# IvanPopov/video-flow-ml

Hardware: AMD Instinct MI355X
Metric: flow-fields/sec @1080p seq5 MOF_sintel (higher is better)
Workload: dtype mixed (per-layer MFMA count, f32 accumulate): {"corr": 1, "update_block.encoder.convf1": 1, "update_block.encoder.convf2": 1, "update_block.gru.convq1.iter": "2a", "update_block.gru.convzr1.iter": 1, "update_block.gru.convzr2.iter": 1, "update_block.mask.0": 1, "update_block.mask.2": 1, "update_bloc

## Files before the change

include/vfml.h:

```cpp
#ifndef VFML_H
#define VFML_H
#include <stddef.h>
#include <stdint.h>

#ifdef __cplusplus
extern "C" {
#endif

#define VFML_ABI_VERSION 26

enum {
  VFML_EPI_NONE = 0,
  VFML_EPI_RELU = 1,
  VFML_EPI_TANH = 2,
  VFML_EPI_SIGMOID = 3,
  VFML_EPI_TANH_RELU = 4,
  VFML_EPI_GRU_ZR = 5,
  VFML_EPI_GRU_Q = 6,
  VFML_EPI_ADD_AUX = 7,
};

enum { VFML_FMT_F32 = 0, VFML_FMT_S16 = 1,
       VFML_FMT_F16 = 2 };

// ... 48 lines not shown

int vfml_add_to_s16(const float* x, int64_t ldx, const float* aux, int64_t ld_aux, float* out, int64_t ld_out, int64_t rows,
                    int c, float scale, void* stream);

int vfml_transpose_split_f16(const float* src, int rows, int c, int ld, float scale, void* hi, void* lo, int kp,
                             void* stream);

int vfml_frames_to_nhwc4(const void* src, int kind, int n, int H, int W,
                         float scale, float shift, float* dst, void* stream);

int64_t vfml_instnorm_workspace_bytes(int n, int hw, int c);
int vfml_instnorm_stats(const float* x, int n, int hw, int c, float eps,
                        float* stats, void* workspace, void* stream);
int vfml_instnorm_apply(const float* x, const float* stats, const float* res,
                        const float* res_stats, int n, int hw, int c, float* out, int out_fmt, void* stream);

int vfml_avgpool2x2(const float* x, int n, int h, int w, int c, float* out, void* stream);

int vfml_corr_lookup(const float* const* pyr, const int32_t* hl, const int32_t* wl,
                     const int32_t* ld, int levels, int radius, int nmaps, int q_per_map,
                     const float* coords, int ld_coords, float* out, int ld_out, int out_fmt, int vol_fmt, int vol_tile,
                     void* stream);
#define VFML_VOL_F16_LEVELS(m) (0x100 | (m))

int vfml_corr_lookup_indirect(const float* const* table, const int32_t* hl, const int32_t* wl, const int32_t* ld,
                              int levels, int radius, int nmaps, int q_per_map, const float* coords, int ld_coords,
                              float* out, int ld_out, int out_fmt, int vol_fmt, int vol_tile, void* stream);
int vfml_corr_lookup_indirect_bidir(const float* const* table, const int32_t* hl, const int32_t* wl, const int32_t* ld,
                                    int levels, int radius, int nmaps, int q_per_map, const float* coords, int ld_coords,
                                    int dir_coords, float* out, int ld_out, int dir_out, int dir_tab, int out_fmt, int vol_fmt,
                                    int vol_tile, void* stream);
int vfml_ptr_table_set(void* table, const void* const* ptrs, int n, void* stream);

#define VFML_SEED_NONE 0
#define VFML_SEED_LOAD 1
#define VFML_SEED_STORE 2
int vfml_window_seed(const void* cells, int ncentres, int rows, int cols, float* state, int ld_state, int h_off, int mf_off,
                     int ld_ctx, void* stream);

int vfml_flow_rows7(const float* flow, int n, int h, int w, float* rows, void* stream);

int vfml_conv3x3_c64(const float* in, int ld_in, int n, int h, int w, const void* w_hi, const void* w_lo, int kp, float w_scale,
                     const float* bias, float* out, int ldo, double* stats_part, void* stream);

int vfml_flow_half(const float* flow, int n, int h, int w, const void* w1_hi, int kp1, float w1_scale, const float* b1,
                   const void* w2_hi, int kp2, float w2_scale, const float* b2, float* out, int ld_out, void* stream);

int vfml_tapsum3x3(const float* t, int ld_t, const float* bias, int n, int h, int w, float* out, int parts, int64_t part_stride,
                   void* stream);
int vfml_tapsum3x3_update(const float* t, int ld_t, const float* bias, int n, int h, int w, int parts, int64_t part_stride,
                          float* coords1, float* flow_a, int ld_a, float* flow_b, int ld_b, int fmt_b, void* stream);

int vfml_coords_update(float* coords1, const float* delta, int n, int h, int w,
                       float* flow_a, int ld_a, float* flow_b, int ld_b, int fmt_b, void* stream);
int vfml_coords_init(float* coords1, int n, int h, int w, void* stream);

int vfml_convex_upsample(const float* coords1, int ch, const float* mask, int ld_mask,
                         int h, int w, float* out, void* stream);
// ... 112 lines not shown
```

video-flow-ml_amd/vfml/csrc/enc_conv.hip:

```cpp
#include "conv_split_common.h"

namespace {

constexpr int EC_C = 64;
constexpr int EC_TH = 4, EC_TW = 32;
constexpr int EC_PR = EC_TH + 2, EC_PW = EC_TW + 2;
constexpr int EC_PIX = 272;
constexpr int EC_PATCH = EC_PR * EC_PW * EC_PIX;
constexpr int EC_VLD = EC_C + 4;
constexpr int EC_LDS = EC_PATCH;
constexpr int EC_K = 9 * EC_C;
constexpr int EC_NS = EC_K / 32;
static_assert(EC_TH * EC_TW * EC_VLD * 4 <= EC_PATCH, "the result tile fits where the patch was");

struct EncConvArgs {
  const char* in;
  const _Float16* whi; const _Float16* wlo;
  const float* bias;
  float* out; int ldo;
  double* stats_part;
  int ld_in, n, H, W, tiles_x, tiles_y;
  float w_inv;
};

__global__ __launch_bounds__(256, 2) void enc_conv3x3_c64_kernel(const EncConvArgs a) {
  extern __shared__ __attribute__((aligned(16))) char smem[];
  float* sV = reinterpret_cast<float*>(smem);

  const int t = threadIdx.x, lane = t & 63;
  const int wave = __builtin_amdgcn_readfirstlane(t >> 6);
  const int r4 = lane & 15, u4 = lane >> 4;
  const int tiles_img = a.tiles_x * a.tiles_y;
  const int total = a.n * tiles_img;

  h16x8 bh[EC_NS], bl[EC_NS];
  static_for<EC_NS>([&](auto sc) {
    constexpr int s = decltype(sc)::value;
    bh[s] = *reinterpret_cast<const h16x8*>(a.whi + (16 * wave + r4) * EC_K + s * 32 + u4 * 8);
    bl[s] = *reinterpret_cast<const h16x8*>(a.wlo + (16 * wave + r4) * EC_K + s * 32 + u4 * 8);
  });
  f32x4 bias4 = {0.f, 0.f, 0.f, 0.f};
  if (a.bias) bias4 = *reinterpret_cast<const f32x4*>(a.bias + 16 * wave + 4 * u4);

  for (int tile = blockIdx.x; tile < total; tile += gridDim.x) {
    const int img = tile / tiles_img, tl = tile - img * tiles_img;
    const int ty = tl / a.tiles_x, tx = tl - ty * a.tiles_x;
    const int oy0 = ty * EC_TH, ox0 = tx * EC_TW;

    constexpr int NPC = EC_PR * EC_PW * 16;
    constexpr int NPT = (NPC + 255) / 256;
    const __amdgpu_buffer_rsrc_t rin = __builtin_amdgcn_make_buffer_rsrc(
        const_cast<char*>(a.in) + (int64_t)img * a.H * a.W * a.ld_in * 4, 0, a.H * a.W * a.ld_in * 4, 0x00020000);
    u32x4 pv[NPT];
    static_for<NPT>([&](auto qc) {
      constexpr int q = decltype(qc)::value;
      const int c = min(t + 256 * q, NPC - 1);
      const int p = c >> 4, piece = c & 15;
      const int py = p / EC_PW, px = p - py * EC_PW;
      const int iy = oy0 - 1 + py, ix = ox0 - 1 + px;
      const bool ok = (unsigned)iy < (unsigned)a.H && (unsigned)ix < (unsigned)a.W;
      pv[q] = bload16(rin, ok ? ((iy * a.W + ix) * a.ld_in) * 4 + piece * 16 : (int)0x80000000);
    });
    __syncthreads();
    static_for<NPT>([&](auto qc) {
      constexpr int q = decltype(qc)::value;
      const int c = t + 256 * q;
      if (c < NPC) *reinterpret_cast<u32x4*>(smem + (c >> 4) * EC_PIX + (c & 15) * 16) = pv[q];
    });
    __syncthreads();

    f32x4 acc[8];
#pragma unroll
    for (int m = 0; m < 8; ++m) acc[m] = f32x4{0.f, 0.f, 0.f, 0.f};
    const char* al = smem + r4 * EC_PIX + u4 * 32;
    static_for<2>([&](auto hc) {
      constexpr int mh = decltype(hc)::value;
      static_for<EC_NS>([&](auto sc) {
        constexpr int s = decltype(sc)::value;
        constexpr int cb = s / 9, ky = (s % 9) / 3, kx = s % 3;
#pragma unroll
        for (int mm = 0; mm < 4; ++mm) {
          const int m = 4 * mh + mm;
// ... 33 lines not shown
          const double v = (double)g;
          s1 += v;
          s2 += v * v;
        }
        const int64_t chunk = (((int64_t)img * a.H + oy) * a.W + ox0) >> 5;
        double* o = a.stats_part + (chunk * EC_C + ch) * 2;
        o[0] = s1;
        o[1] = s2;
      }
    }
  }
}

}

extern "C" int vfml_conv3x3_c64(const float* in, int ld_in, int n, int h, int w, const void* w_hi, const void* w_lo, int kp,
                                float w_scale, const float* bias, float* out, int ldo, double* stats_part, void* stream) {
  VFML_REQUIRE(in && w_hi && w_lo && out && n > 0 && h > 0 && w > 0, "vfml_conv3x3_c64: bad argument");
  VFML_REQUIRE(w % EC_TW == 0, "vfml_conv3x3_c64: the image width must be a multiple of %d (got %d)", EC_TW, w);
  VFML_REQUIRE(kp == EC_K && w_scale > 0.f, "vfml_conv3x3_c64: weight planes [64][%d] (VFML_KORDER_CBLOCK), got row pitch %d", EC_K, kp);
  VFML_REQUIRE((reinterpret_cast<uintptr_t>(in) & 31u) == 0 && ld_in >= EC_C && ld_in % 8 == 0 && vfml_aligned16(w_hi) &&
                   vfml_aligned16(w_lo) && vfml_aligned16(bias) && vfml_aligned16(out) && ldo >= EC_C && ldo % 4 == 0 &&
                   (reinterpret_cast<uintptr_t>(stats_part) & 7u) == 0,
               "vfml_conv3x3_c64: a 32-byte aligned split-row input (ld_in %% 8 == 0), 16-byte aligned weights / bias / output "
               "(ldo %% 4 == 0)");
  EncConvArgs a;
  a.in = reinterpret_cast<const char*>(in); a.ld_in = ld_in;
  a.whi = reinterpret_cast<const _Float16*>(w_hi); a.wlo = reinterpret_cast<const _Float16*>(w_lo);
  a.bias = bias; a.out = out; a.ldo = ldo; a.stats_part = stats_part;
  a.n = n; a.H = h; a.W = w; a.tiles_x = w / EC_TW; a.tiles_y = (h + EC_TH - 1) / EC_TH;
  a.w_inv = 1.0f / w_scale;
  const int64_t total = (int64_t)n * a.tiles_x * a.tiles_y;
  VFML_REQUIRE(total < (1ll << 31) && (int64_t)h * w * ld_in * 4 < (1ll << 31), "vfml_conv3x3_c64: an image of the input must stay below 2 GiB");
  const int grid = (int)(total < 512 ? total : 512);
  hipLaunchKernelGGL(enc_conv3x3_c64_kernel, dim3(grid), dim3(256), EC_LDS, reinterpret_cast<hipStream_t>(stream), a);
  return vfml_check_launch("vfml_conv3x3_c64");
}
```

video-flow-ml_amd/vfml/csrc/norm_pool.hip:

```cpp
#include <stdlib.h>
#include "vfml_common.h"

namespace {

__global__ void frames_u8_kernel(const uint8_t* __restrict__ src, int64_t npx, float scale, float shift,
                                 f32x4* __restrict__ dst) {
  for (int64_t p = (int64_t)blockIdx.x * blockDim.x + threadIdx.x; p < npx; p += (int64_t)gridDim.x * blockDim.x) {
    const uint8_t* s = src + p * 3;
    f32x4 v;
    v[0] = scale * ((float)s[0] / 255.0f) + shift;
    v[1] = scale * ((float)s[1] / 255.0f) + shift;
    v[2] = scale * ((float)s[2] / 255.0f) + shift;
    v[3] = 0.f;
    dst[p] = v;
  }
}

__global__ void frames_f32_kernel(const float* __restrict__ src, int n, int64_t hw, float scale, float shift,
                                  f32x4* __restrict__ dst) {
  const int64_t npx = (int64_t)n * hw;
  for (int64_t p = (int64_t)blockIdx.x * blockDim.x + threadIdx.x; p < npx; p += (int64_t)gridDim.x * blockDim.x) {
    const int64_t f = p / hw, q = p - f * hw;
    const float* s = src + f * 3 * hw + q;
    f32x4 v;
// ... 121 lines not shown
    double* o = out + (((int64_t)nn * FOLD_SLICES + sl) * c + cg * 8 + ch) * 2;
    o[0] = ss;
    o[1] = qq;
  }
}

template <int MODE, bool S16>
__global__ void instnorm_apply_kernel(const f32x4* __restrict__ x, const float* __restrict__ stats,
                                      const f32x4* __restrict__ res, const float* __restrict__ rstats, int hw, int c,
                                      int64_t total4, f32x4* __restrict__ out) {
  const int cg = c >> 2;
  const int64_t per_n = (int64_t)hw * cg;
  for (int64_t i = (int64_t)blockIdx.x * blockDim.x + threadIdx.x; i < total4; i += (int64_t)gridDim.x * blockDim.x) {
    const int n = (int)(i / per_n);
    const int g = (int)(i % cg);
    const float* st = stats + ((int64_t)n * c + g * 4) * 2;
    const f32x4 v = x[i];
    f32x4 o;
#pragma unroll
    for (int e = 0; e < 4; ++e) o[e] = fmaxf((v[e] - st[2 * e]) * st[2 * e + 1], 0.f);
    const int64_t qoff = (i - g) * 16 + (g >> 1) * 32 + (g & 1) * 8;
    if (MODE == 1) {
      f32x4 rv;
      if (S16) {
        const char* u = reinterpret_cast<const char*>(res) + qoff;
        const vfml_h16x2 h0 = *reinterpret_cast<const vfml_h16x2*>(u), h1 = *reinterpret_cast<const vfml_h16x2*>(u + 4);
        const vfml_h16x2 l0 = *reinterpret_cast<const vfml_h16x2*>(u + 16), l1 = *reinterpret_cast<const vfml_h16x2*>(u + 20);
        rv[0] = (float)h0[0] + (float)l0[0];
        rv[1] = (float)h0[1] + (float)l0[1];
        rv[2] = (float)h1[0] + (float)l1[0];
        rv[3] = (float)h1[1] + (float)l1[1];
      } else {
        rv = res[i];
      }
#pragma unroll
      for (int e = 0; e < 4; ++e) o[e] = fmaxf(rv[e] + o[e], 0.f);
    } else if (MODE == 2) {
      const f32x4 rv = res[i];
      const float* rs = rstats + ((int64_t)n * c + g * 4) * 2;
#pragma unroll
      for (int e = 0; e < 4; ++e) o[e] = fmaxf((rv[e] - rs[2 * e]) * rs[2 * e + 1] + o[e], 0.f);
    }
    if (S16) {
      vfml_h16x2 h0, h1, l0, l1;
      vfml_split2(o[0], o[1], h0, l0);
      vfml_split2(o[2], o[3], h1, l1);
      char* u = reinterpret_cast<char*>(out) + qoff;
      uint2 hv, lv;
      hv.x = __builtin_bit_cast(unsigned, h0); hv.y = __builtin_bit_cast(unsigned, h1);
      lv.x = __builtin_bit_cast(unsigned, l0); lv.y = __builtin_bit_cast(unsigned, l1);
      *reinterpret_cast<uint2*>(u) = hv;
      *reinterpret_cast<uint2*>(u + 16) = lv;
    } else {
      out[i] = o;
    }
  }
}

__global__ void avgpool2x2_kernel(const f32x4* __restrict__ x, int h, int w, int cg, int ho, int wo, int64_t total4,
                                  f32x4* __restrict__ out) {
  for (int64_t i = (int64_t)blockIdx.x * blockDim.x + threadIdx.x; i < total4; i += (int64_t)gridDim.x * blockDim.x) {
    const int g = (int)(i % cg);
    int64_t p = i / cg;
    const int ox = (int)(p % wo);
    p /= wo;
    const int oy = (int)(p % ho);
    const int n = (int)(p / ho);
// ... 103 lines not shown
  const bool s16 = out_fmt == VFML_FMT_S16;
#define VFML_APPLY(MODE, S16, R, RS)                                                                                      \
  hipLaunchKernelGGL((instnorm_apply_kernel<MODE, S16>), g, b, 0, s, (const f32x4*)x, stats, (const f32x4*)(R), RS, hw, c, \
                     total4, (f32x4*)out)
  if (!res) {
    if (s16) VFML_APPLY(0, true, nullptr, nullptr); else VFML_APPLY(0, false, nullptr, nullptr);
  } else if (!res_stats) {
    if (s16) VFML_APPLY(1, true, res, nullptr); else VFML_APPLY(1, false, res, nullptr);
  } else {
    if (s16) VFML_APPLY(2, true, res, res_stats); else VFML_APPLY(2, false, res, res_stats);
  }
#undef VFML_APPLY
  return vfml_check_launch("vfml_instnorm_apply");
}

extern "C" int vfml_avgpool2x2(const float* x, int n, int h, int w, int c, float* out, void* stream) {
  VFML_REQUIRE(x && out, "vfml_avgpool2x2: null pointer");
  VFML_REQUIRE(n > 0 && h >= 2 && w >= 2 && c > 0 && c % 4 == 0, "vfml_avgpool2x2: bad shape");
  VFML_REQUIRE(vfml_aligned16(x) && vfml_aligned16(out), "vfml_avgpool2x2: alignment");
  const int ho = h / 2, wo = w / 2, cg = c / 4;
  const int64_t total4 = (int64_t)n * ho * wo * cg;
  hipLaunchKernelGGL(avgpool2x2_kernel, dim3(grid_for(total4, 256)), dim3(256), 0, reinterpret_cast<hipStream_t>(stream),
                     (const f32x4*)x, h, w, cg, ho, wo, total4, (f32x4*)out);
  return vfml_check_launch("vfml_avgpool2x2");
}
```

video-flow-ml_amd/vfml/csrc/vfml_common.h:

```cpp
#pragma once
#include <hip/hip_runtime.h>
#include <stdint.h>
#include <stdio.h>
#include <mutex>
#include <set>
#include <utility>
#include "../../../include/vfml.h"

typedef float f32x4 __attribute__((ext_vector_type(4)));
typedef float f32x16 __attribute__((ext_vector_type(16)));

typedef _Float16 vfml_h16x2 __attribute__((ext_vector_type(2)));

__device__ __forceinline__ void vfml_split2(float a, float b, vfml_h16x2& h, vfml_h16x2& l) {
  vfml_h16x2 hh = {(_Float16)a, (_Float16)b};
#if defined(__HIP_DEVICE_COMPILE__)
  unsigned hp = __builtin_bit_cast(unsigned, hh);
  asm volatile("" : "+v"(hp));
  hh = __builtin_bit_cast(vfml_h16x2, hp);
#endif
  h = hh;
  const vfml_h16x2 ll = {(_Float16)(a - (float)hh[0]), (_Float16)(b - (float)hh[1])};
  l = ll;
}

__device__ __forceinline__ double vfml_lds_f64(const double* p) {
#if defined(__HIP_DEVICE_COMPILE__)
  const uint2 u = *reinterpret_cast<const uint2*>(p);
  unsigned lo, hi;
  asm("v_mov_b32 %0, %1" : "=v"(lo) : "v"(u.x));
  asm("v_mov_b32 %0, %1" : "=v"(hi) : "v"(u.y));
  return __hiloint2double((int)hi, (int)lo);
#else
  return *p;
#endif
}

void vfml_set_error(const char* fmt, ...);
// ... 38 lines not shown
```

video-flow-ml_amd/vfml/hip.py:

```python
import ctypes
import os
import subprocess
from ctypes import POINTER, c_char_p, c_double, c_float, c_int, c_int32, c_int64, c_void_p

import torch

_HERE = os.path.dirname(os.path.abspath(__file__))
LIB_PATH = os.environ.get("VFML_LIB") or os.path.join(_HERE, "libvfml_hip.so")
CSRC = os.path.join(_HERE, "csrc")
SOURCES = ["api.hip", "conv_gemm.hip", "conv_gemm_split.hip", "conv_gemm_tapx.hip", "conv_split_plan.hip", "stem.hip", "flow_half.hip", "enc_conv.hip", "norm_pool.hip", "flow_ops.hip", "effects.hip", "correct.hip", "render.hip", "turbulence.hip", "resize.hip", "jpeg.hip", "jpeg_decode.hip", "jpeg_decode_sync.hip", "deflate.hip"]

STATS_ROWS_F32, STATS_ROWS_S16 = 128, 32
EPI_NONE, EPI_RELU, EPI_TANH, EPI_SIGMOID, EPI_TANH_RELU, EPI_GRU_ZR, EPI_GRU_Q, EPI_ADD_AUX = range(8)
FMT_F32, FMT_S16, FMT_F16 = 0, 1, 2


def vol_f16_levels(mask):
    return 0x100 | mask


def _vol_mask(vol_fmt, levels):
    return (15 if vol_fmt == FMT_F16 else (vol_fmt & 15 if vol_fmt & 0x100 else 0)) & ((1 << levels) - 1)

KORDER_TAP, KORDER_CBLOCK, KORDER_CBLOCK64 = 0, 1, 2
# ... 83 lines not shown
    L.vfml_transpose_split_f16.argtypes = [c_void_p, c_int, c_int, c_int, c_float, c_void_p, c_void_p, c_int, c_void_p]
    L.vfml_split_f16.argtypes = [c_void_p, c_int64, c_int, c_int, c_float, c_void_p, c_void_p, c_int, c_void_p]
    L.vfml_frames_to_nhwc4.argtypes = [c_void_p, c_int, c_int, c_int, c_int, c_float, c_float, c_void_p, c_void_p]
    L.vfml_instnorm_workspace_bytes.restype = c_int64
    L.vfml_instnorm_workspace_bytes.argtypes = [c_int, c_int, c_int]
    L.vfml_instnorm_stats.argtypes = [c_void_p, c_int, c_int, c_int, c_float, c_void_p, c_void_p, c_void_p]
    L.vfml_softmax_rows_f16.argtypes = [c_void_p, c_int64, c_int, c_int64, c_void_p, c_int64, c_float, c_void_p]
    L.vfml_transpose_to_s16.argtypes = [c_void_p, c_int, c_int, c_int, c_float, c_void_p, c_int64, c_void_p]
    L.vfml_add_to_s16.argtypes = [c_void_p, c_int64, c_void_p, c_int64, c_void_p, c_int64, c_int64, c_int, c_float, c_void_p]
    L.vfml_instnorm_finalize.argtypes = [c_void_p, c_int, c_int, c_int, c_int, c_float, c_void_p, c_void_p, c_int64, c_void_p]
    L.vfml_instnorm_finalize_workspace_bytes.restype = c_int64
    L.vfml_instnorm_finalize_workspace_bytes.argtypes = [c_int, c_int]
    L.vfml_stem7x7s2_chunks.argtypes = [c_int, c_int]
    L.vfml_stem7x7s2.argtypes = [c_void_p, c_int, c_int, c_int, c_void_p, c_void_p, c_float, c_void_p, c_void_p, c_void_p, c_void_p]
    L.vfml_instnorm_apply.argtypes = [c_void_p, c_void_p, c_void_p, c_void_p, c_int, c_int, c_int, c_void_p, c_int, c_void_p]
    L.vfml_avgpool2x2.argtypes = [c_void_p, c_int, c_int, c_int, c_int, c_void_p, c_void_p]
    L.vfml_corr_lookup.argtypes = [POINTER(c_void_p), POINTER(c_int32), POINTER(c_int32), POINTER(c_int32),
                                   c_int, c_int, c_int, c_int, c_void_p, c_int, c_void_p, c_int, c_int, c_int, c_int, c_void_p]
    L.vfml_corr_lookup_indirect.argtypes = [c_void_p, POINTER(c_int32), POINTER(c_int32), POINTER(c_int32),
                                            c_int, c_int, c_int, c_int, c_void_p, c_int, c_void_p, c_int, c_int, c_int, c_int,
                                            c_void_p]
    L.vfml_corr_lookup_indirect_bidir.argtypes = [c_void_p, POINTER(c_int32), POINTER(c_int32), POINTER(c_int32),
                                                  c_int, c_int, c_int, c_int, c_void_p, c_int, c_int, c_void_p, c_int, c_int,
                                                  c_int, c_int, c_int, c_int, c_void_p]
    L.vfml_ptr_table_set.argtypes = [c_void_p, POINTER(c_void_p), c_int, c_void_p]
    L.vfml_window_seed.argtypes = [c_void_p, c_int, c_int, c_int, c_void_p, c_int, c_int, c_int, c_int, c_void_p]
    L.vfml_tapsum3x3_update.argtypes = [c_void_p, c_int, c_void_p, c_int, c_int, c_int, c_int, ctypes.c_int64, c_void_p, c_void_p,
                                        c_int, c_void_p, c_int, c_int, c_void_p]
    L.vfml_conv3x3_c64.argtypes = [c_void_p, c_int, c_int, c_int, c_int, c_void_p, c_void_p, c_int, c_float, c_void_p, c_void_p,
                                   c_int, c_void_p, c_void_p]
    L.vfml_flow_half.argtypes = [c_void_p, c_int, c_int, c_int, c_void_p, c_int, c_float, c_void_p, c_void_p, c_int, c_float,
                                 c_void_p, c_void_p, c_int, c_void_p]
    L.vfml_coords_init.argtypes = [c_void_p, c_int, c_int, c_int, c_void_p]
    L.vfml_flow_rows7.argtypes = [c_void_p, c_int, c_int, c_int, c_void_p, c_void_p]
    L.vfml_tapsum3x3.argtypes = [c_void_p, c_int, c_void_p, c_int, c_int, c_int, c_void_p, c_int, ctypes.c_int64, c_void_p]
    L.vfml_coords_update.argtypes = [c_void_p, c_void_p, c_int, c_int, c_int, c_void_p, c_int, c_void_p, c_int,
                                     c_int, c_void_p]
    L.vfml_flow_lod.argtypes = [c_void_p, c_int, c_int, c_void_p, c_void_p]
    L.vfml_flow_encode.argtypes = [c_void_p, c_int, c_int, c_int, c_float, c_float, c_float, c_float, c_float, c_void_p,
                                   c_void_p]
    L.vfml_taa_blend.argtypes = [c_void_p, c_int, c_void_p, c_void_p, c_int, c_void_p, c_int, c_int, c_int, c_int, c_double,
                                 c_double, c_void_p]
    L.vfml_flow_quality_map.argtypes = [c_void_p, c_void_p, c_void_p, c_int, c_int, c_int, c_int, c_float, c_void_p, c_void_p]
    L.vfml_flow_correct_workspace_bytes.argtypes = [c_int, c_int]
    L.vfml_flow_correct_workspace_bytes.restype = ctypes.c_size_t
# ... 42 lines not shown
                                      c_void_p, c_void_p, c_void_p]
    L.vfml_convex_upsample.argtypes = [c_void_p, c_int, c_void_p, c_int, c_int, c_int, c_void_p, c_void_p]
    for name in EXPORTS:
        getattr(L, name)
    if L.vfml_abi_version() != 26:
        raise RuntimeError("libvfml_hip.so ABI version mismatch")
    _lib = L
    return L


EXPORTS = [
    "vfml_conv2d", "vfml_conv2d_split", "vfml_conv2d_variant", "vfml_conv2d_split_variant", "vfml_split_f16", "vfml_to_s16", "vfml_softmax_rows_s16", "vfml_softmax_rows_f16", "vfml_transpose_to_s16", "vfml_add_to_s16",
    "vfml_transpose_split_f16", "vfml_frames_to_nhwc4", "vfml_instnorm_workspace_bytes", "vfml_instnorm_stats",
    "vfml_instnorm_apply", "vfml_instnorm_finalize", "vfml_instnorm_finalize_workspace_bytes", "vfml_avgpool2x2", "vfml_corr_lookup", "vfml_corr_lookup_indirect", "vfml_corr_lookup_indirect_bidir",
    "vfml_ptr_table_set", "vfml_window_seed", "vfml_coords_update", "vfml_coords_init", "vfml_tapsum3x3", "vfml_tapsum3x3_update", "vfml_flow_rows7", "vfml_flow_half", "vfml_conv3x3_c64",
    "vfml_convex_upsample", "vfml_stem7x7s2", "vfml_stem7x7s2_chunks", "vfml_flow_lod", "vfml_flow_encode", "vfml_taa_blend", "vfml_flow_quality_map", "vfml_flow_correct_workspace_bytes", "vfml_flow_correct",
    "vfml_flow_colorize", "vfml_compose_frame", "vfml_flow_decode", "vfml_flow_diff_overlay",
    "vfml_flow_turbulence_workspace_bytes", "vfml_flow_turbulence_map", "vfml_resize_u8",
    "vfml_jpeg_workspace_bytes", "vfml_jpeg_scan_capacity", "vfml_jpeg_encode_rgb",
    "vfml_jpeg_decode_workspace_bytes", "vfml_jpeg_decode_rgb",
    "vfml_jpeg_decode_sync_workspace_bytes", "vfml_jpeg_decode_rgb_sync",
    "vfml_jpeg_decode_sampled_workspace_bytes", "vfml_jpeg_decode_rgb_sampled",
    "vfml_jpeg_decode_sync_sampled_workspace_bytes", "vfml_jpeg_decode_rgb_sync_sampled",
    "vfml_deflate_capacity", "vfml_deflate_workspace_bytes", "vfml_deflate_huffman",
    "vfml_inflate_workspace_bytes", "vfml_inflate_chunks",
    "vfml_last_error", "vfml_abi_version",
]


def _check(rc, what):
# ... 214 lines not shown
        raise ValueError(f"pack_stem_weight: a [64, 3|4, 7, 7] weight expected, got {tuple(w.shape)}")
    k = torch.zeros(cout, 7, 8, 4, device=device)
    k[:, :, :7, :cin] = w.permute(0, 2, 3, 1)
    sw = SplitWeight(cout, 224, device)
    return sw.fill(k.reshape(-1).contiguous(), scale=SplitWeight.auto_scale(float(w.abs().max())))


def stem7x7s2(frames, n, h, w, weight, bias, out, stats_part=None):
    if not isinstance(weight, SplitWeight) or weight.rows != 64 or weight.kp != 224:
        raise ValueError("stem7x7s2: weight must come from pack_stem_weight")
    _check(lib().vfml_stem7x7s2(_ptr(_dev(frames)), n, h, w, c_void_p(weight.hi.data_ptr()), c_void_p(weight.lo.data_ptr()),
                                weight.scale, _ptr(_dev(bias)) if bias is not None else None, _ptr(_dev(out)),
                                c_void_p(stats_part.data_ptr()) if stats_part is not None else None, _stream()), "vfml_stem7x7s2")


def instnorm_apply(x, stats, n, hw, c, out, res=None, res_stats=None, out_fmt=FMT_F32):
    _check(lib().vfml_instnorm_apply(_ptr(_dev(x)), _ptr(_dev(stats)), _ptr(res), _ptr(res_stats), n, hw, c,
                                     _ptr(_dev(out)), out_fmt, _stream()), "vfml_instnorm_apply")


def avgpool2x2(x, n, h, w, c, out):
    _check(lib().vfml_avgpool2x2(_ptr(_dev(x)), n, h, w, c, _ptr(_dev(out)), _stream()), "vfml_avgpool2x2")


def softmax_rows_s16(x, rows, cols, ld_in, out, ld_out, x_off=0, out_off=0, scale=1.0):
    _check(lib().vfml_softmax_rows_s16(_ptr(_dev(x), x_off), rows, cols, ld_in, _ptr(_dev(out), out_off), ld_out,
                                       float(scale), _stream()), "vfml_softmax_rows_s16")


class PlainWeight:
    lo = None
# ... 120 lines not shown
def flow_rows7(flow, n, h, w, rows):
    _check(lib().vfml_flow_rows7(_ptr(_dev(flow)), n, h, w, _ptr(_dev(rows)), _stream()), "vfml_flow_rows7")


def tapsum3x3(t, ld_t, bias, n, h, w, out, parts=1, part_stride=0):
    _check(lib().vfml_tapsum3x3(_ptr(_dev(t)), ld_t, _ptr(bias) if bias is not None else None, n, h, w, _ptr(_dev(out)),
                                parts, part_stride, _stream()), "vfml_tapsum3x3")


def conv3x3_c64(src, ld_in, n, h, w, weight, bias, out, ldo, stats_part=None, src_off=0):
    _check(lib().vfml_conv3x3_c64(_ptr(_dev(src), src_off), ld_in, n, h, w, c_void_p(weight.hi.data_ptr()),
                                  c_void_p(weight.lo.data_ptr()), weight.kp, weight.scale,
                                  _ptr(_dev(bias)) if bias is not None else None, _ptr(_dev(out)), ldo,
                                  c_void_p(stats_part.data_ptr()) if stats_part is not None else None, _stream()),
           "vfml_conv3x3_c64")


def flow_half(flow, n, h, w, w1, b1, w2, b2, out, ld_out, out_off=0):
    _check(lib().vfml_flow_half(_ptr(_dev(flow)), n, h, w, c_void_p(w1.hi.data_ptr()), w1.kp, w1.scale, _ptr(_dev(b1)),
                                c_void_p(w2.hi.data_ptr()), w2.kp, w2.scale, _ptr(_dev(b2)), _ptr(_dev(out), out_off), ld_out,
                                _stream()), "vfml_flow_half")


def tapsum3x3_update(t, ld_t, bias, n, h, w, coords1, parts=1, part_stride=0, flow_a=None, ld_a=0, flow_a_off=0, flow_b=None,
                     ld_b=0, flow_b_off=0, fmt_b=FMT_F32):
    _check(lib().vfml_tapsum3x3_update(_ptr(_dev(t)), ld_t, _ptr(bias) if bias is not None else None, n, h, w, parts, part_stride,
                                       _ptr(_dev(coords1)), _ptr(flow_a, flow_a_off), ld_a, _ptr(flow_b, flow_b_off), ld_b,
                                       fmt_b, _stream()), "vfml_tapsum3x3_update")


# ... 551 lines not shown
```

video-flow-ml_amd/vfml/network.py:

```python
import os

import torch
import torch.nn as nn

from . import hip
from .weights import conv_spec, corr_channel_subset, pack_conv_weight


def cor_pad(cor, split):
    return (cor + 15) // 16 * 16 if split else (cor + 3) // 4 * 4


def take_frames(src, idx):
    idx = list(idx)
    if all(b == a + 1 for a, b in zip(idx, idx[1:])):
        return src[idx[0]:idx[0] + len(idx)]
    return torch.stack([src[i] for i in idx])


class _Holder(nn.Module):

    def child(self, name):
        if name not in self._modules:
            self.add_module(name, _Holder())
# ... 330 lines not shown
            return
        st = self._graphs.get(key)
        if st is None:
            body()
            while len(self._graphs) >= self.GRAPHS_KEPT:
                self._graphs.pop(next(iter(self._graphs)))
            self._graphs[key] = "seen"
            return
        if st == "seen":
            g = torch.cuda.CUDAGraph()
            with torch.cuda.graph(g, capture_error_mode="thread_local"):
                body()
            self._graphs[key] = st = g
        st.replay()

    def _encoder(self, prefix, x, n, H, W, P, dev, out, ldo, out_off, epilogue, split, out_fmt=hip.FMT_F32):
        h2, w2 = H // 2, W // 2
        big = n * h2 * w2 * 64
        raw = self._buf("enc_raw", big, dev)
        raw2 = self._buf("enc_raw2", big, dev)
        act = [self._buf("enc_act0", big, dev), self._buf("enc_act1", big, dev), self._buf("enc_act2", big, dev)]
        st = self._buf("enc_stats", 3 * n * 128 * 2, dev)
        nws = hip.instnorm_workspace_bytes(n, h2 * w2, 128)
        ws = self._buf("enc_statws", (nws + 7) // 8, dev, torch.float64)

        def stats_of(t, hw, c, slot):
            s = st[slot * n * 128 * 2:]
            hip.instnorm_stats(t, n, hw, c, s, ws)
            return s

        split_prec = self._split()
        AF = hip.FMT_S16 if split_prec else hip.FMT_F32
        part_len = n * ((h2 * w2 + 31) // 32) * 64 * 2
        parts = self._buf("enc_part", 3 * part_len, dev, torch.float64) if split_prec else None
        fold_ws = self._buf("enc_foldws", min(n, 8) * 64 * 128 * 2, dev, torch.float64) if split_prec else None

        def conv_stats(src, c, hh_, ww_, name, planes, dst, slot, k, stride=1, pad=0, src_fmt=hip.FMT_F32):
            wgt, b = P[name]
            nm = self._nm(name) if split_prec else 3
            ho_, wo_ = (hh_ + 2 * pad - k) // stride + 1, (ww_ + 2 * pad - k) // stride + 1
            hw = ho_ * wo_
            rows = hip.STATS_ROWS_S16 if src_fmt == hip.FMT_S16 else hip.STATS_ROWS_F32
            if not (split_prec and (n == 1 or hw % rows == 0)):
                hip.conv2d(src, c, c, n, hh_, ww_, wgt, b, planes, k, k, dst, planes, stride=stride, pad_h=pad, pad_w=pad,
                           mfma=nm, in_fmt=src_fmt)
                return stats_of(dst, hw, planes, slot)
            chunks = (hw + rows - 1) // rows
            part = parts[slot * part_len:]
            if (c == 64 and planes == 64 and k == 3 and stride == 1 and pad == 1 and nm == 3 and src_fmt == hip.FMT_S16
                    and ww_ % 32 == 0 and getattr(wgt, "order", None) == hip.KORDER_CBLOCK and wgt.kp == 576 and wgt.lo is not None):
                hip.conv3x3_c64(src, c, n, hh_, ww_, wgt, b, dst, planes, stats_part=part)
            else:
                hip.conv2d(src, c, c, n, hh_, ww_, wgt, b, planes, k, k, dst, planes, stride=stride, pad_h=pad, pad_w=pad,
                           stats_part=part, mfma=nm, in_fmt=src_fmt)
            s = st[slot * n * 128 * 2:]
            hip.instnorm_finalize(part, n, chunks, planes, hw, s, workspace=fold_ws)
            return s

        stem = P.get(f"{prefix}.conv1.stem")
        if stem is not None and split_prec and self._nm(f"{prefix}.conv1") == 3:
            chunks = hip.stem_chunks(H, W)
            part = parts[0:]
            hip.stem7x7s2(x, n, H, W, stem[0], stem[1], raw, stats_part=part)
            s0 = st[0:]
            hip.instnorm_finalize(part, n, chunks, 64, h2 * w2, s0, workspace=fold_ws)
        else:
            s0 = conv_stats(x, 4, H, W, f"{prefix}.conv1", 64, raw, 0, 7, stride=2, pad=3)
        cur = act[0]
        hip.instnorm_apply(raw, s0, n, h2 * w2, 64, cur, out_fmt=AF)
        ch, hh, ww, ci = 64, h2, w2, 0
        for li, (planes, stride) in enumerate([(64, 1), (96, 2), (128, 2)], start=1):
            for bi in range(2):
                stv = stride if bi == 0 else 1
                ho, wo = (hh, ww) if stv == 1 else ((hh - 1) // 2 + 1, (ww - 1) // 2 + 1)
                name = f"{prefix}.layer{li}.{bi}"
                y = act[(ci + 1) % 3]
                nxt = act[(ci + 2) % 3]
                s1 = conv_stats(cur, ch, hh, ww, f"{name}.conv1", planes, raw, 0, 3, stride=stv, pad=1, src_fmt=AF)
                hip.instnorm_apply(raw, s1, n, ho * wo, planes, y, out_fmt=AF)
                s2 = conv_stats(y, planes, ho, wo, f"{name}.conv2", planes, raw, 1, 3, pad=1, src_fmt=AF)
                if stv != 1:
                    s3 = conv_stats(cur, ch, hh, ww, f"{name}.downsample.0", planes, raw2, 2, 1, stride=stv, src_fmt=AF)
                    hip.instnorm_apply(raw, s2, n, ho * wo, planes, nxt, res=raw2, res_stats=s3, out_fmt=AF)
                else:
                    hip.instnorm_apply(raw, s2, n, ho * wo, planes, nxt, res=cur, out_fmt=AF)
                cur, ci = nxt, (ci + 2) % 3
# ... 519 lines not shown
```

Measured before the change: 44.76.

## Fuse instance-norm+ReLU into encoder layer1 conv input loads

Adds a templated NORM variant of the 64-channel 3x3 encoder conv. It applies instance-norm and ReLU to raw fp32 inputs while staging them into LDS, splitting them into f16 hi/lo halves and zeroing the padding. The encoder's layer1 path now feeds raw conv outputs plus their stats straight into the next conv, and a new apply variant normalises the residual on the fly. This removes three standalone instnorm_apply passes over the activation map, at the cost of reading fp32 (twice the bytes of split storage) in the conv and extra ALU work in its load phase.

Result: no change. 45.12, median of 6 (+0.8%).

```diff
diff --git a/include/vfml.h b/include/vfml.h
--- a/include/vfml.h
+++ b/include/vfml.h
@@ -86,6 +86,8 @@
                         float* stats, void* workspace, void* stream);
 int vfml_instnorm_apply(const float* x, const float* stats, const float* res,
                         const float* res_stats, int n, int hw, int c, float* out, int out_fmt, void* stream);
+int vfml_instnorm_apply_normres(const float* x, const float* stats, const float* res, const float* res_stats, int n, int hw,
+                                int c, float* out, void* stream);
 
 int vfml_avgpool2x2(const float* x, int n, int h, int w, int c, float* out, void* stream);
 
@@ -114,6 +116,9 @@
 
 int vfml_conv3x3_c64(const float* in, int ld_in, int n, int h, int w, const void* w_hi, const void* w_lo, int kp, float w_scale,
                      const float* bias, float* out, int ldo, double* stats_part, void* stream);
+int vfml_conv3x3_c64_norm(const float* in, const float* in_stats, int ld_in, int n, int h, int w, const void* w_hi,
+                          const void* w_lo, int kp, float w_scale, const float* bias, float* out, int ldo, double* stats_part,
+                          void* stream);
 
 int vfml_flow_half(const float* flow, int n, int h, int w, const void* w1_hi, int kp1, float w1_scale, const float* b1,
                    const void* w2_hi, int kp2, float w2_scale, const float* b2, float* out, int ld_out, void* stream);
diff --git a/video-flow-ml_amd/vfml/csrc/enc_conv.hip b/video-flow-ml_amd/vfml/csrc/enc_conv.hip
--- a/video-flow-ml_amd/vfml/csrc/enc_conv.hip
+++ b/video-flow-ml_amd/vfml/csrc/enc_conv.hip
@@ -15,6 +15,7 @@
 
 struct EncConvArgs {
   const char* in;
+  const float* nstats;
   const _Float16* whi; const _Float16* wlo;
   const float* bias;
   float* out; int ldo;
@@ -23,6 +24,7 @@
   float w_inv;
 };
 
+template <bool NORM>
 __global__ __launch_bounds__(256, 2) void enc_conv3x3_c64_kernel(const EncConvArgs a) {
   extern __shared__ __attribute__((aligned(16))) char smem[];
   float* sV = reinterpret_cast<float*>(smem);
@@ -52,20 +54,37 @@
     const __amdgpu_buffer_rsrc_t rin = __builtin_amdgcn_make_buffer_rsrc(
         const_cast<char*>(a.in) + (int64_t)img * a.H * a.W * a.ld_in * 4, 0, a.H * a.W * a.ld_in * 4, 0x00020000);
     u32x4 pv[NPT];
+    unsigned inside = 0;
+    int ts = t;
+    if (NORM) asm volatile("" : "+v"(ts));
     static_for<NPT>([&](auto qc) {
       constexpr int q = decltype(qc)::value;
-      const int c = min(t + 256 * q, NPC - 1);
+      const int c = min(ts + 256 * q, NPC - 1);
       const int p = c >> 4, piece = c & 15;
       const int py = p / EC_PW, px = p - py * EC_PW;
       const int iy = oy0 - 1 + py, ix = ox0 - 1 + px;
       const bool ok = (unsigned)iy < (unsigned)a.H && (unsigned)ix < (unsigned)a.W;
       pv[q] = bload16(rin, ok ? ((iy * a.W + ix) * a.ld_in) * 4 + piece * 16 : (int)0x80000000);
+      if (NORM) inside |= (unsigned)ok << q;
     });
+    f32x4 mean = {0.f, 0.f, 0.f, 0.f}, rstd = mean;
+    if (NORM) vfml_load_stats4(a.nstats + ((int64_t)img * EC_C + 4 * (t & 15)) * 2, mean, rstd);
     __syncthreads();
     static_for<NPT>([&](auto qc) {
       constexpr int q = decltype(qc)::value;
       const int c = t + 256 * q;
-      if (c < NPC) *reinterpret_cast<u32x4*>(smem + (c >> 4) * EC_PIX + (c & 15) * 16) = pv[q];
+      if (c < NPC) {
+        if (NORM) {
+          vfml_s16quad s = vfml_norm_relu_split4(__builtin_bit_cast(f32x4, pv[q]), mean, rstd);
+          const unsigned keep = 0u - (inside >> q & 1u);
+          s.hi.x &= keep; s.hi.y &= keep; s.lo.x &= keep; s.lo.y &= keep;
+          char* u = smem + (c >> 4) * EC_PIX + ((c & 15) >> 1) * 32 + (c & 1) * 8;
+          *reinterpret_cast<uint2*>(u) = s.hi;
+          *reinterpret_cast<uint2*>(u + 16) = s.lo;
+        } else {
+          *reinterpret_cast<u32x4*>(smem + (c >> 4) * EC_PIX + (c & 15) * 16) = pv[q];
+        }
+      }
     });
     __syncthreads();
 
@@ -129,25 +148,43 @@
 
 }
 
-extern "C" int vfml_conv3x3_c64(const float* in, int ld_in, int n, int h, int w, const void* w_hi, const void* w_lo, int kp,
-                                float w_scale, const float* bias, float* out, int ldo, double* stats_part, void* stream) {
-  VFML_REQUIRE(in && w_hi && w_lo && out && n > 0 && h > 0 && w > 0, "vfml_conv3x3_c64: bad argument");
-  VFML_REQUIRE(w % EC_TW == 0, "vfml_conv3x3_c64: the image width must be a multiple of %d (got %d)", EC_TW, w);
-  VFML_REQUIRE(kp == EC_K && w_scale > 0.f, "vfml_conv3x3_c64: weight planes [64][%d] (VFML_KORDER_CBLOCK), got row pitch %d", EC_K, kp);
+static int enc_conv_launch(const char* who, bool norm, const float* in, const float* stats, int ld_in, int n, int h, int w,
+                           const void* w_hi, const void* w_lo, int kp, float w_scale, const float* bias, float* out, int ldo,
+                           double* stats_part, void* stream) {
+  VFML_REQUIRE(in && w_hi && w_lo && out && (stats || !norm) && n > 0 && h > 0 && w > 0, "%s: bad argument (null pointer or empty shape)", who);
+  VFML_REQUIRE(w % EC_TW == 0, "%s: the image width must be a multiple of %d (got %d)", who, EC_TW, w);
+  VFML_REQUIRE(kp == EC_K && w_scale > 0.f, "%s: weight planes [64][%d] (VFML_KORDER_CBLOCK), got row pitch %d", who, EC_K, kp);
   VFML_REQUIRE((reinterpret_cast<uintptr_t>(in) & 31u) == 0 && ld_in >= EC_C && ld_in % 8 == 0 && vfml_aligned16(w_hi) &&
                    vfml_aligned16(w_lo) && vfml_aligned16(bias) && vfml_aligned16(out) && ldo >= EC_C && ldo % 4 == 0 &&
                    (reinterpret_cast<uintptr_t>(stats_part) & 7u) == 0,
-               "vfml_conv3x3_c64: a 32-byte aligned split-row input (ld_in %% 8 == 0), 16-byte aligned weights / bias / output "
-               "(ldo %% 4 == 0)");
+               "%s: a 32-byte aligned input (ld_in %% 8 == 0), 16-byte aligned weights / bias / output (ldo %% 4 == 0)", who);
+  VFML_REQUIRE(vfml_aligned16(stats), "%s: the input's statistics must be 16-byte aligned", who);
+  VFML_REQUIRE(!norm || in != out, "%s: the output must not be the map it reads", who);
   EncConvArgs a;
-  a.in = reinterpret_cast<const char*>(in); a.ld_in = ld_in;
+  a.in = reinterpret_cast<const char*>(in); a.nstats = stats; a.ld_in = ld_in;
   a.whi = reinterpret_cast<const _Float16*>(w_hi); a.wlo = reinterpret_cast<const _Float16*>(w_lo);
   a.bias = bias; a.out = out; a.ldo = ldo; a.stats_part = stats_part;
   a.n = n; a.H = h; a.W = w; a.tiles_x = w / EC_TW; a.tiles_y = (h + EC_TH - 1) / EC_TH;
   a.w_inv = 1.0f / w_scale;
   const int64_t total = (int64_t)n * a.tiles_x * a.tiles_y;
-  VFML_REQUIRE(total < (1ll << 31) && (int64_t)h * w * ld_in * 4 < (1ll << 31), "vfml_conv3x3_c64: an image of the input must stay below 2 GiB");
+  VFML_REQUIRE(total < (1ll << 31) && (int64_t)h * w * ld_in * 4 < (1ll << 31), "%s: an image of the input must stay below 2 GiB", who);
   const int grid = (int)(total < 512 ? total : 512);
-  hipLaunchKernelGGL(enc_conv3x3_c64_kernel, dim3(grid), dim3(256), EC_LDS, reinterpret_cast<hipStream_t>(stream), a);
-  return vfml_check_launch("vfml_conv3x3_c64");
+  if (norm)
+    hipLaunchKernelGGL(enc_conv3x3_c64_kernel<true>, dim3(grid), dim3(256), EC_LDS, reinterpret_cast<hipStream_t>(stream), a);
+  else
+    hipLaunchKernelGGL(enc_conv3x3_c64_kernel<false>, dim3(grid), dim3(256), EC_LDS, reinterpret_cast<hipStream_t>(stream), a);
+  return vfml_check_launch(who);
 }
+
+extern "C" int vfml_conv3x3_c64(const float* in, int ld_in, int n, int h, int w, const void* w_hi, const void* w_lo, int kp,
+                                float w_scale, const float* bias, float* out, int ldo, double* stats_part, void* stream) {
+  return enc_conv_launch("vfml_conv3x3_c64", false, in, nullptr, ld_in, n, h, w, w_hi, w_lo, kp, w_scale, bias, out, ldo, stats_part,
+                         stream);
+}
+
+extern "C" int vfml_conv3x3_c64_norm(const float* in, const float* in_stats, int ld_in, int n, int h, int w, const void* w_hi,
+                                     const void* w_lo, int kp, float w_scale, const float* bias, float* out, int ldo,
+                                     double* stats_part, void* stream) {
+  return enc_conv_launch("vfml_conv3x3_c64_norm", true, in, in_stats, ld_in, n, h, w, w_hi, w_lo, kp, w_scale, bias, out, ldo,
+                         stats_part, stream);
+}
diff --git a/video-flow-ml_amd/vfml/csrc/norm_pool.hip b/video-flow-ml_amd/vfml/csrc/norm_pool.hip
--- a/video-flow-ml_amd/vfml/csrc/norm_pool.hip
+++ b/video-flow-ml_amd/vfml/csrc/norm_pool.hip
@@ -159,22 +159,22 @@
   for (int64_t i = (int64_t)blockIdx.x * blockDim.x + threadIdx.x; i < total4; i += (int64_t)gridDim.x * blockDim.x) {
     const int n = (int)(i / per_n);
     const int g = (int)(i % cg);
-    const float* st = stats + ((int64_t)n * c + g * 4) * 2;
-    const f32x4 v = x[i];
-    f32x4 o;
-#pragma unroll
-    for (int e = 0; e < 4; ++e) o[e] = fmaxf((v[e] - st[2 * e]) * st[2 * e + 1], 0.f);
+    f32x4 mean, rstd;
+    vfml_load_stats4(stats + ((int64_t)n * c + g * 4) * 2, mean, rstd);
+    f32x4 o = vfml_norm_relu4(x[i], mean, rstd);
     const int64_t qoff = (i - g) * 16 + (g >> 1) * 32 + (g & 1) * 8;
-    if (MODE == 1) {
+    if (MODE == 1 || MODE == 3) {
       f32x4 rv;
-      if (S16) {
+      if (MODE == 3) {
+        f32x4 rmean, rrstd;
+        vfml_load_stats4(rstats + ((int64_t)n * c + g * 4) * 2, rmean, rrstd);
+        rv = vfml_join4(vfml_norm_relu_split4(res[i], rmean, rrstd));
+      } else if (S16) {
         const char* u = reinterpret_cast<const char*>(res) + qoff;
-        const vfml_h16x2 h0 = *reinterpret_cast<const vfml_h16x2*>(u), h1 = *reinterpret_cast<const vfml_h16x2*>(u + 4);
-        const vfml_h16x2 l0 = *reinterpret_cast<const vfml_h16x2*>(u + 16), l1 = *reinterpret_cast<const vfml_h16x2*>(u + 20);
-        rv[0] = (float)h0[0] + (float)l0[0];
-        rv[1] = (float)h0[1] + (float)l0[1];
-        rv[2] = (float)h1[0] + (float)l1[0];
-        rv[3] = (float)h1[1] + (float)l1[1];
+        vfml_s16quad q;
+        q.hi = *reinterpret_cast<const uint2*>(u);
+        q.lo = *reinterpret_cast<const uint2*>(u + 16);
+        rv = vfml_join4(q);
       } else {
         rv = res[i];
       }
@@ -187,15 +187,10 @@
       for (int e = 0; e < 4; ++e) o[e] = fmaxf((rv[e] - rs[2 * e]) * rs[2 * e + 1] + o[e], 0.f);
     }
     if (S16) {
-      vfml_h16x2 h0, h1, l0, l1;
-      vfml_split2(o[0], o[1], h0, l0);
-      vfml_split2(o[2], o[3], h1, l1);
+      const vfml_s16quad q = vfml_split4(o);
       char* u = reinterpret_cast<char*>(out) + qoff;
-      uint2 hv, lv;
-      hv.x = __builtin_bit_cast(unsigned, h0); hv.y = __builtin_bit_cast(unsigned, h1);
-      lv.x = __builtin_bit_cast(unsigned, l0); lv.y = __builtin_bit_cast(unsigned, l1);
-      *reinterpret_cast<uint2*>(u) = hv;
-      *reinterpret_cast<uint2*>(u + 16) = lv;
+      *reinterpret_cast<uint2*>(u) = q.hi;
+      *reinterpret_cast<uint2*>(u + 16) = q.lo;
     } else {
       out[i] = o;
     }
@@ -329,6 +324,21 @@
   return vfml_check_launch("vfml_instnorm_apply");
 }
 
+extern "C" int vfml_instnorm_apply_normres(const float* x, const float* stats, const float* res, const float* res_stats, int n,
+                                           int hw, int c, float* out, void* stream) {
+  VFML_REQUIRE(x && stats && res && res_stats && out, "vfml_instnorm_apply_normres: null pointer");
+  VFML_REQUIRE(n > 0 && hw > 0 && c > 0 && c % 8 == 0, "vfml_instnorm_apply_normres: bad n/hw/c (c %% 8 == 0)");
+  VFML_REQUIRE(vfml_aligned16(x) && vfml_aligned16(res) && (reinterpret_cast<uintptr_t>(out) & 31u) == 0,
+               "vfml_instnorm_apply_normres: 16-byte aligned x and res, 32-byte aligned split-row out");
+  VFML_REQUIRE(vfml_aligned16(stats) && vfml_aligned16(res_stats),
+               "vfml_instnorm_apply_normres: stats and res_stats must be 16-byte aligned");
+  const int64_t total4 = (int64_t)n * hw * (c / 4);
+  hipLaunchKernelGGL((instnorm_apply_kernel<3, true>), dim3(grid_for(total4, 256)), dim3(256), 0,
+                     reinterpret_cast<hipStream_t>(stream), (const f32x4*)x, stats, (const f32x4*)res, res_stats, hw, c,
+                     total4, (f32x4*)out);
+  return vfml_check_launch("vfml_instnorm_apply_normres");
+}
+
 extern "C" int vfml_avgpool2x2(const float* x, int n, int h, int w, int c, float* out, void* stream) {
   VFML_REQUIRE(x && out, "vfml_avgpool2x2: null pointer");
   VFML_REQUIRE(n > 0 && h >= 2 && w >= 2 && c > 0 && c % 4 == 0, "vfml_avgpool2x2: bad shape");
diff --git a/video-flow-ml_amd/vfml/csrc/vfml_common.h b/video-flow-ml_amd/vfml/csrc/vfml_common.h
--- a/video-flow-ml_amd/vfml/csrc/vfml_common.h
+++ b/video-flow-ml_amd/vfml/csrc/vfml_common.h
@@ -22,6 +22,48 @@
   h = hh;
   const vfml_h16x2 ll = {(_Float16)(a - (float)hh[0]), (_Float16)(b - (float)hh[1])};
   l = ll;
+}
+
+struct vfml_s16quad { uint2 hi, lo; };
+
+__device__ __forceinline__ f32x4 vfml_norm_relu4(const f32x4 v, const f32x4 mean, const f32x4 rstd) {
+  f32x4 o;
+#pragma unroll
+  for (int e = 0; e < 4; ++e) o[e] = fmaxf((v[e] - mean[e]) * rstd[e], 0.f);
+  return o;
+}
+
+__device__ __forceinline__ vfml_s16quad vfml_split4(const f32x4 o) {
+  vfml_h16x2 h0, h1, l0, l1;
+  vfml_split2(o[0], o[1], h0, l0);
+  vfml_split2(o[2], o[3], h1, l1);
+  vfml_s16quad q;
+  q.hi.x = __builtin_bit_cast(unsigned, h0); q.hi.y = __builtin_bit_cast(unsigned, h1);
+  q.lo.x = __builtin_bit_cast(unsigned, l0); q.lo.y = __builtin_bit_cast(unsigned, l1);
+  return q;
+}
+
+__device__ __forceinline__ f32x4 vfml_join4(const vfml_s16quad q) {
+  const vfml_h16x2 h0 = __builtin_bit_cast(vfml_h16x2, q.hi.x), h1 = __builtin_bit_cast(vfml_h16x2, q.hi.y);
+  const vfml_h16x2 l0 = __builtin_bit_cast(vfml_h16x2, q.lo.x), l1 = __builtin_bit_cast(vfml_h16x2, q.lo.y);
+  f32x4 r;
+  r[0] = (float)h0[0] + (float)l0[0];
+  r[1] = (float)h0[1] + (float)l0[1];
+  r[2] = (float)h1[0] + (float)l1[0];
+  r[3] = (float)h1[1] + (float)l1[1];
+  return r;
+}
+
+__device__ __forceinline__ vfml_s16quad vfml_norm_relu_split4(const f32x4 v, const f32x4 mean, const f32x4 rstd) {
+  return vfml_split4(vfml_norm_relu4(v, mean, rstd));
+}
+
+__device__ __forceinline__ void vfml_load_stats4(const float* st, f32x4& mean, f32x4& rstd) {
+#pragma unroll
+  for (int e = 0; e < 4; ++e) {
+    mean[e] = st[2 * e];
+    rstd[e] = st[2 * e + 1];
+  }
 }
 
 __device__ __forceinline__ double vfml_lds_f64(const double* p) {
diff --git a/video-flow-ml_amd/vfml/hip.py b/video-flow-ml_amd/vfml/hip.py
--- a/video-flow-ml_amd/vfml/hip.py
+++ b/video-flow-ml_amd/vfml/hip.py
@@ -121,6 +121,7 @@
     L.vfml_stem7x7s2_chunks.argtypes = [c_int, c_int]
     L.vfml_stem7x7s2.argtypes = [c_void_p, c_int, c_int, c_int, c_void_p, c_void_p, c_float, c_void_p, c_void_p, c_void_p, c_void_p]
     L.vfml_instnorm_apply.argtypes = [c_void_p, c_void_p, c_void_p, c_void_p, c_int, c_int, c_int, c_void_p, c_int, c_void_p]
+    L.vfml_instnorm_apply_normres.argtypes = [c_void_p, c_void_p, c_void_p, c_void_p, c_int, c_int, c_int, c_void_p, c_void_p]
     L.vfml_avgpool2x2.argtypes = [c_void_p, c_int, c_int, c_int, c_int, c_void_p, c_void_p]
     L.vfml_corr_lookup.argtypes = [POINTER(c_void_p), POINTER(c_int32), POINTER(c_int32), POINTER(c_int32),
                                    c_int, c_int, c_int, c_int, c_void_p, c_int, c_void_p, c_int, c_int, c_int, c_int, c_void_p]
@@ -136,6 +137,8 @@
                                         c_int, c_void_p, c_int, c_int, c_void_p]
     L.vfml_conv3x3_c64.argtypes = [c_void_p, c_int, c_int, c_int, c_int, c_void_p, c_void_p, c_int, c_float, c_void_p, c_void_p,
                                    c_int, c_void_p, c_void_p]
+    L.vfml_conv3x3_c64_norm.argtypes = [c_void_p, c_void_p, c_int, c_int, c_int, c_int, c_void_p, c_void_p, c_int, c_float, c_void_p,
+                                        c_void_p, c_int, c_void_p, c_void_p]
     L.vfml_flow_half.argtypes = [c_void_p, c_int, c_int, c_int, c_void_p, c_int, c_float, c_void_p, c_void_p, c_int, c_float,
                                  c_void_p, c_void_p, c_int, c_void_p]
     L.vfml_coords_init.argtypes = [c_void_p, c_int, c_int, c_int, c_void_p]
@@ -208,6 +211,7 @@
     "vfml_transpose_split_f16", "vfml_frames_to_nhwc4", "vfml_instnorm_workspace_bytes", "vfml_instnorm_stats",
     "vfml_instnorm_apply", "vfml_instnorm_finalize", "vfml_instnorm_finalize_workspace_bytes", "vfml_avgpool2x2", "vfml_corr_lookup", "vfml_corr_lookup_indirect", "vfml_corr_lookup_indirect_bidir",
     "vfml_ptr_table_set", "vfml_window_seed", "vfml_coords_update", "vfml_coords_init", "vfml_tapsum3x3", "vfml_tapsum3x3_update", "vfml_flow_rows7", "vfml_flow_half", "vfml_conv3x3_c64",
+    "vfml_conv3x3_c64_norm", "vfml_instnorm_apply_normres",
     "vfml_convex_upsample", "vfml_stem7x7s2", "vfml_stem7x7s2_chunks", "vfml_flow_lod", "vfml_flow_encode", "vfml_taa_blend", "vfml_flow_quality_map", "vfml_flow_correct_workspace_bytes", "vfml_flow_correct",
     "vfml_flow_colorize", "vfml_compose_frame", "vfml_flow_decode", "vfml_flow_diff_overlay",
     "vfml_flow_turbulence_workspace_bytes", "vfml_flow_turbulence_map", "vfml_resize_u8",
@@ -452,7 +456,13 @@
                                 c_void_p(stats_part.data_ptr()) if stats_part is not None else None, _stream()), "vfml_stem7x7s2")
 
 
-def instnorm_apply(x, stats, n, hw, c, out, res=None, res_stats=None, out_fmt=FMT_F32):
+def instnorm_apply(x, stats, n, hw, c, out, res=None, res_stats=None, out_fmt=FMT_F32, res_relu_split=False):
+    if res_relu_split:
+        if out_fmt != FMT_S16 or res is None or res_stats is None:
+            raise ValueError("instnorm_apply: res_relu_split needs res, res_stats and a split-row out")
+        _check(lib().vfml_instnorm_apply_normres(_ptr(_dev(x)), _ptr(_dev(stats)), _ptr(_dev(res)), _ptr(_dev(res_stats)), n, hw,
+                                                 c, _ptr(_dev(out)), _stream()), "vfml_instnorm_apply_normres")
+        return
     _check(lib().vfml_instnorm_apply(_ptr(_dev(x)), _ptr(_dev(stats)), _ptr(res), _ptr(res_stats), n, hw, c,
                                      _ptr(_dev(out)), out_fmt, _stream()), "vfml_instnorm_apply")
 
@@ -603,6 +613,14 @@
                                   _ptr(_dev(bias)) if bias is not None else None, _ptr(_dev(out)), ldo,
                                   c_void_p(stats_part.data_ptr()) if stats_part is not None else None, _stream()),
            "vfml_conv3x3_c64")
+
+
+def conv3x3_c64_norm(src, src_stats, ld_in, n, h, w, weight, bias, out, ldo, stats_part=None):
+    _check(lib().vfml_conv3x3_c64_norm(_ptr(_dev(src)), _ptr(_dev(src_stats)), ld_in, n, h, w, c_void_p(weight.hi.data_ptr()),
+                                       c_void_p(weight.lo.data_ptr()), weight.kp, weight.scale,
+                                       _ptr(_dev(bias)) if bias is not None else None, _ptr(_dev(out)), ldo,
+                                       c_void_p(stats_part.data_ptr()) if stats_part is not None else None, _stream()),
+           "vfml_conv3x3_c64_norm")
 
 
 def flow_half(flow, n, h, w, w1, b1, w2, b2, out, ld_out, out_off=0):
diff --git a/video-flow-ml_amd/vfml/network.py b/video-flow-ml_amd/vfml/network.py
--- a/video-flow-ml_amd/vfml/network.py
+++ b/video-flow-ml_amd/vfml/network.py
@@ -368,13 +368,15 @@
             self._graphs[key] = st = g
         st.replay()
 
+    enc_norm_on_load = True
+
     def _encoder(self, prefix, x, n, H, W, P, dev, out, ldo, out_off, epilogue, split, out_fmt=hip.FMT_F32):
         h2, w2 = H // 2, W // 2
         big = n * h2 * w2 * 64
         raw = self._buf("enc_raw", big, dev)
         raw2 = self._buf("enc_raw2", big, dev)
         act = [self._buf("enc_act0", big, dev), self._buf("enc_act1", big, dev), self._buf("enc_act2", big, dev)]
-        st = self._buf("enc_stats", 3 * n * 128 * 2, dev)
+        st = self._buf("enc_stats", 4 * n * 128 * 2, dev)
         nws = hip.instnorm_workspace_bytes(n, h2 * w2, 128)
         ws = self._buf("enc_statws", (nws + 7) // 8, dev, torch.float64)
 
@@ -389,21 +391,29 @@
         parts = self._buf("enc_part", 3 * part_len, dev, torch.float64) if split_prec else None
         fold_ws = self._buf("enc_foldws", min(n, 8) * 64 * 128 * 2, dev, torch.float64) if split_prec else None
 
-        def conv_stats(src, c, hh_, ww_, name, planes, dst, slot, k, stride=1, pad=0, src_fmt=hip.FMT_F32):
+        def c64_route(name, ww_):
+            wgt = P[name][0]
+            return (self._nm(name) == 3 and ww_ % 32 == 0 and getattr(wgt, "order", None) == hip.KORDER_CBLOCK and wgt.kp == 576
+                    and wgt.lo is not None)
+
+        def conv_stats(src, c, hh_, ww_, name, planes, dst, slot, k, stride=1, pad=0, src_fmt=hip.FMT_F32, src_stats=None):
             wgt, b = P[name]
             nm = self._nm(name) if split_prec else 3
             ho_, wo_ = (hh_ + 2 * pad - k) // stride + 1, (ww_ + 2 * pad - k) // stride + 1
             hw = ho_ * wo_
             rows = hip.STATS_ROWS_S16 if src_fmt == hip.FMT_S16 else hip.STATS_ROWS_F32
+            assert src_stats is None or (split_prec and (n == 1 or hw % rows == 0))
             if not (split_prec and (n == 1 or hw % rows == 0)):
                 hip.conv2d(src, c, c, n, hh_, ww_, wgt, b, planes, k, k, dst, planes, stride=stride, pad_h=pad, pad_w=pad,
                            mfma=nm, in_fmt=src_fmt)
                 return stats_of(dst, hw, planes, slot)
             chunks = (hw + rows - 1) // rows
-            part = parts[slot * part_len:]
-            if (c == 64 and planes == 64 and k == 3 and stride == 1 and pad == 1 and nm == 3 and src_fmt == hip.FMT_S16
-                    and ww_ % 32 == 0 and getattr(wgt, "order", None) == hip.KORDER_CBLOCK and wgt.kp == 576 and wgt.lo is not None):
-                hip.conv3x3_c64(src, c, n, hh_, ww_, wgt, b, dst, planes, stats_part=part)
+            part = parts[slot % 3 * part_len:]
+            if c == 64 and planes == 64 and k == 3 and stride == 1 and pad == 1 and src_fmt == hip.FMT_S16 and c64_route(name, ww_):
+                if src_stats is not None:
+                    hip.conv3x3_c64_norm(src, src_stats, c, n, hh_, ww_, wgt, b, dst, planes, stats_part=part)
+                else:
+                    hip.conv3x3_c64(src, c, n, hh_, ww_, wgt, b, dst, planes, stats_part=part)
             else:
                 hip.conv2d(src, c, c, n, hh_, ww_, wgt, b, planes, k, k, dst, planes, stride=stride, pad_h=pad, pad_w=pad,
                            stats_part=part, mfma=nm, in_fmt=src_fmt)
@@ -416,14 +426,28 @@
             chunks = hip.stem_chunks(H, W)
             part = parts[0:]
             hip.stem7x7s2(x, n, H, W, stem[0], stem[1], raw, stats_part=part)
-            s0 = st[0:]
+            s0 = st[3 * n * 128 * 2:]
             hip.instnorm_finalize(part, n, chunks, 64, h2 * w2, s0, workspace=fold_ws)
         else:
-            s0 = conv_stats(x, 4, H, W, f"{prefix}.conv1", 64, raw, 0, 7, stride=2, pad=3)
-        cur = act[0]
-        hip.instnorm_apply(raw, s0, n, h2 * w2, 64, cur, out_fmt=AF)
-        ch, hh, ww, ci = 64, h2, w2, 0
-        for li, (planes, stride) in enumerate([(64, 1), (96, 2), (128, 2)], start=1):
+            s0 = conv_stats(x, 4, H, W, f"{prefix}.conv1", 64, raw, 3, 7, stride=2, pad=3)
+        ch, hh, ww = 64, h2, w2
+        layers = [(1, 64, 1), (2, 96, 2), (3, 128, 2)]
+        l1 = [f"{prefix}.layer1.{bi}.conv{k}" for bi in (0, 1) for k in (1, 2)]
+        if (self.enc_norm_on_load and split_prec and (n == 1 or hh * ww % hip.STATS_ROWS_S16 == 0)
+                and all(c64_route(name, ww) for name in l1)):
+            s1 = conv_stats(raw, 64, hh, ww, l1[0], 64, raw2, 0, 3, pad=1, src_fmt=AF, src_stats=s0)
+            s2 = conv_stats(raw2, 64, hh, ww, l1[1], 64, act[1], 1, 3, pad=1, src_fmt=AF, src_stats=s1)
+            cur = act[2]
+            hip.instnorm_apply(act[1], s2, n, hh * ww, 64, cur, res=raw, res_stats=s0, out_fmt=AF, res_relu_split=True)
+            s1 = conv_stats(cur, 64, hh, ww, l1[2], 64, raw, 0, 3, pad=1, src_fmt=AF)
+            s2 = conv_stats(raw, 64, hh, ww, l1[3], 64, raw2, 1, 3, pad=1, src_fmt=AF, src_stats=s1)
+            hip.instnorm_apply(raw2, s2, n, hh * ww, 64, act[1], res=cur, out_fmt=AF)
+            cur, ci = act[1], 1
+            layers = layers[1:]
+        else:
+            cur, ci = act[0], 0
+            hip.instnorm_apply(raw, s0, n, h2 * w2, 64, cur, out_fmt=AF)
+        for li, planes, stride in layers:
             for bi in range(2):
                 stv = stride if bi == 0 else 1
                 ho, wo = (hh, ww) if stv == 1 else ((hh - 1) // 2 + 1, (ww - 1) // 2 + 1)
```
